# intel/hdk

Measured on AMD Instinct MI355X. Metric: rows/sec, 1B-row int64 GROUP BY SUM, higher is better.
Workload: dtype int64; 1 GPU; C2: SELECT key, SUM(val) GROUP BY key; int64, 64 uniform keys; rows=1000000000, rows_per_gpu=1000000000, fragments=32, fragments_per_gpu=32, fragment_rows=32000000, layout=perfect hash, keyless, 64 entries, parallelism=fragment f -> GPU f mod 1; one GPU

## Files before the change

### hdk_amd/_lib.py

```python
import ctypes as C
import os
import subprocess

from . import _abi as A

_HERE = os.path.dirname(os.path.abspath(__file__))
LIB_PATH = os.environ.get("HDK_HIP_LIB") or os.path.join(_HERE, "libhdk_hip.so")
CSRC = os.path.join(_HERE, "csrc")


class HdkHipError(RuntimeError):
    def __init__(self, code, msg):
        super().__init__(f"hdk_hip status {code}: {msg}")
        self.code = code


def build(force=False):
    if force:
        subprocess.check_call(["make", "-C", CSRC, "clean"])
    subprocess.check_call(["make", "-C", CSRC, "-j4"])
    return LIB_PATH


_lib = None
# ... 116 lines not shown
                          f"{LIB_PATH} is missing: run `python -c 'import __graft_entry__ as g; g.build()'` "
                          "(make -C hdk_amd/csrc).  There is no CPU fallback.")
    _share_hip_runtime_with_torch()
    L = C.CDLL(LIB_PATH)
    for name, (res, args) in {**SIGNATURES, **EXTRA_SIGNATURES}.items():
        f = getattr(L, name)
        f.restype = res
        f.argtypes = args
    _lib = L
    return L


_switch_env = None


def sync_switches():
    global _switch_env
    now = tuple(sorted((k, v) for k, v in os.environ.items() if k.startswith("HDK_HIP_")))
    if now != _switch_env:
        lib().hdk_hip_reload_switches()
        _switch_env = now


def check(status: int):
    if status != A.OK:
        msg = lib().hdk_hip_last_error()
        raise HdkHipError(status, msg.decode() if msg else "")
    return status
```

### hdk_amd/csrc/host_common.h

```cpp
#pragma once
#include <hip/hip_runtime.h>
#include <stdarg.h>
#include <stdint.h>
#include <stdio.h>

#include "../../include/hdk_hip.h"

namespace hdk {

void set_error(const char* fmt, ...);
void clear_error();
int32_t device_enter(int32_t device_id, void* stream, hipStream_t* out);
const hdk_hip_device_properties* device_props(int32_t device_id);
const int32_t* device_interrupt_word(int32_t device_id);
enum ScanPer { SCAN_PER_4 = 4, SCAN_PER_16 = 16 };
void launch_counts_scan(uint32_t* counts, uint32_t n, ScanPer per, uint64_t* total_out, hipStream_t s);
int32_t launch_init_row_wise_indirect(int64_t* const* groupby_buf, const int64_t* init_vals, uint32_t entry_count,
                                      uint32_t key_count, uint32_t key_width, uint32_t row_size_quad, int keyless,
                                      const hdk_hip_device_properties* props, hipStream_t s);
inline int32_t init_row_wise_output(const hdk_hip_plan* plan, int64_t* const* groupby_buf, const int64_t* init_vals,
                                    const hdk_hip_device_properties* props, hipStream_t s) {
  const uint32_t key_count = plan->keyless ? 0u : static_cast<uint32_t>(plan->key_count);
  return launch_init_row_wise_indirect(groupby_buf, init_vals, plan->entry_count, key_count, static_cast<uint32_t>(plan->key_width),
                                       plan->row_size_quad, plan->keyless, props, s);
}

#define HDK_HIP_CHECK(expr)                                                                  \
  do {                                                                                       \
    hipError_t e_ = (expr);                                                                  \
    if (e_ != hipSuccess) {                                                                  \
      hdk::set_error("%s failed: %s (%s:%d)", #expr, hipGetErrorString(e_), __FILE__, __LINE__); \
      return e_ == hipErrorOutOfMemory ? HDK_HIP_ERR_OUT_OF_GPU_MEM : HDK_HIP_ERR_RUNTIME;   \
    }                                                                                        \
  } while (0)

#define HDK_REQUIRE(cond, ...)          \
  do {                                  \
// ... 51 lines not shown
```

### hdk_amd/csrc/reduce.hip

```cpp
#include <mutex>
#include <string.h>

#include "baseline_table.h"
#include "device_common.h"
#include "group_buffer.h"
#include "host_common.h"

namespace hdk {

constexpr int kPlanCacheSlots = 16;
struct PlanCacheEntry {
  hdk_hip_plan host;
  hdk_hip_plan* dev = nullptr;
  bool used = false;
};
struct PlanCache {
  std::mutex mu;
  PlanCacheEntry e[kPlanCacheSlots];
  int next = 0;
};
static PlanCache g_plan_cache[16];

static int32_t cached_device_plan(const hdk_hip_plan* plan, int32_t device_id, const hdk_hip_plan** out) {
  PlanCache& c = g_plan_cache[device_id & 15];
  std::lock_guard<std::mutex> lk(c.mu);
  for (int i = 0; i < kPlanCacheSlots; ++i) {
    if (c.e[i].used && memcmp(&c.e[i].host, plan, sizeof(hdk_hip_plan)) == 0) {
      *out = c.e[i].dev;
      return HDK_HIP_OK;
    }
  }
  PlanCacheEntry& e = c.e[c.next];
  c.next = (c.next + 1) % kPlanCacheSlots;
  if (!e.dev) {
    HDK_HIP_CHECK(hipMalloc(reinterpret_cast<void**>(&e.dev), sizeof(hdk_hip_plan)));
  }
  e.used = false;
  HDK_HIP_CHECK(hipDeviceSynchronize());
  HDK_HIP_CHECK(hipMemcpy(e.dev, plan, sizeof(hdk_hip_plan), hipMemcpyHostToDevice));
  memcpy(&e.host, plan, sizeof(hdk_hip_plan));
  e.used = true;
  *out = e.dev;
  return HDK_HIP_OK;
}

constexpr int kRedBlock = 256;
HDK_DEV bool reduce_single_value(const hdk_hip_target& tg, int8_t* this1, const int8_t* that1, int64_t init_val) {
  if (tg.slot_width == 4) {
    const int32_t l = *reinterpret_cast<const int32_t*>(this1), r = *reinterpret_cast<const int32_t*>(that1);
    if (r == static_cast<int32_t>(init_val)) return false;
    if (l == static_cast<int32_t>(init_val)) {
      *reinterpret_cast<int32_t*>(this1) = r;
      return false;
    }
    return l != r;
  }
  const int64_t l = *reinterpret_cast<const int64_t*>(this1), r = *reinterpret_cast<const int64_t*>(that1);
  if (r == init_val) return false;
  if (l == init_val) {
    *reinterpret_cast<int64_t*>(this1) = r;
    return false;
  }
  return l != r;
}

HDK_DEV void reduce_slot(const hdk_hip_target& tg, int8_t* this1, int8_t* this2, const int8_t* that1,
                         const int8_t* that2, int64_t init_val) {
// ... 356 lines not shown
    nslots += p->targets[t].agg == HDK_AGG_AVG ? 2 : 1;
  }
  size_t off = p->keyless ? 0 : static_cast<size_t>(p->key_count) * ((static_cast<size_t>(entry_count) * 8 + 7) & ~size_t(7));
  int s = 0;
  for (int t = 0; t < p->num_targets && s < nslots; ++t) {
    off = (off + 7) & ~size_t(7);
    off += static_cast<size_t>(entry_count) * p->targets[t].slot_width;
    ++s;
    if (p->targets[t].agg == HDK_AGG_AVG) {
      off = (off + 7) & ~size_t(7);
      off += static_cast<size_t>(entry_count) * p->targets[t].slot2_width;
      ++s;
    }
  }
  return ((off + 7) & ~size_t(7)) / 8;
}

template <int MODE>
static int32_t run_partition(const hdk_hip_plan* plan, const int64_t* buf, uint32_t entry_count, const int64_t* init_vals,
                             int32_t num_owners, uint32_t* counts_out, const OwnerSegs& segs, int32_t device_id,
                             hipStream_t s) {
  SlotInit init;
  fill_slot_init(plan, init_vals, &init);
  AsyncScratch mem(s);
  constexpr size_t kPlanBytes = align256(sizeof(hdk_hip_plan));
  HDK_HIP_CHECK(hipMallocAsync(&mem.p, kPlanBytes + kMaxOwners * sizeof(uint32_t), s));
  int8_t* scratch = static_cast<int8_t*>(mem.p);
  hdk_hip_plan* d_plan = reinterpret_cast<hdk_hip_plan*>(scratch);
  uint32_t* cursors = reinterpret_cast<uint32_t*>(scratch + kPlanBytes);
  HDK_HIP_CHECK(hipMemcpyAsync(d_plan, plan, sizeof(hdk_hip_plan), hipMemcpyHostToDevice, s));
  HDK_HIP_CHECK(hipMemsetAsync(cursors, 0, kMaxOwners * sizeof(uint32_t), s));
  const hdk_hip_device_properties* props = device_props(device_id);
  unsigned blocks = persistent_grid(props, (static_cast<size_t>(entry_count) + kRedBlock * kPartT - 1) / (kRedBlock * kPartT));
  if (blocks == 0) blocks = 1;
  const bool k32 = !plan->output_columnar && plan->key_width == 4;
  if (k32) {
    hipLaunchKernelGGL((k_partition_baseline<int32_t, MODE>), dim3(blocks), dim3(kRedBlock), 0, s,
                       d_plan, buf, entry_count, static_cast<uint32_t>(num_owners), init, cursors, segs);
  } else {
    hipLaunchKernelGGL((k_partition_baseline<int64_t, MODE>), dim3(blocks), dim3(kRedBlock), 0, s,
                       d_plan, buf, entry_count, static_cast<uint32_t>(num_owners), init, cursors, segs);
  }
  HDK_HIP_CHECK(hipGetLastError());
  if (counts_out) {
    HDK_HIP_CHECK(hipMemcpyAsync(counts_out, cursors, num_owners * sizeof(uint32_t), hipMemcpyDeviceToHost, s));
    HDK_HIP_CHECK(hipStreamSynchronize(s));
  }
  return HDK_HIP_OK;
}

int32_t validate_plan_layout(const hdk_hip_plan* p);

}
// ... 118 lines not shown
```

### hdk_amd/csrc/runtime.hip

```cpp
#include <algorithm>
#include <mutex>
#include <stdlib.h>
#include <string.h>

#include "host_common.h"
#include "switches.h"

namespace hdk {
namespace {
constexpr int kSwitchLen = 64;
const char* const kSwitchNames[SW_COUNT] = {
#define HDK_SW_NAME(name) "HDK_HIP_" #name,
    HDK_SWITCH_LIST(HDK_SW_NAME)
#undef HDK_SW_NAME
};
struct SwitchTable {
  bool set[SW_COUNT];
  char val[SW_COUNT][kSwitchLen];
};
SwitchTable g_switches;
std::once_flag g_switches_once;
void read_switches() {
  for (int i = 0; i < SW_COUNT; ++i) {
    const char* e = getenv(kSwitchNames[i]);
// ... 93 lines not shown
  std::call_once(g_dev[d].once, init_device, d);
  if (g_dev[d].status != HDK_HIP_OK) {
    set_error("failed to initialise device %d", d);
  }
  return g_dev[d].status;
}

int32_t device_enter(int32_t device_id, void* stream, hipStream_t* out) {
  const int32_t st = ensure_device(device_id);
  if (st != HDK_HIP_OK) {
    return st;
  }
  HDK_HIP_CHECK(hipSetDevice(device_id));
  *out = stream ? static_cast<hipStream_t>(stream) : g_dev[device_id].stream;
  return HDK_HIP_OK;
}

const hdk_hip_device_properties* device_props(int32_t device_id) {
  return ensure_device(device_id) == HDK_HIP_OK ? &g_dev[device_id].props : nullptr;
}

const int32_t* device_interrupt_word(int32_t device_id) {
  return ensure_device(device_id) == HDK_HIP_OK ? g_dev[device_id].interrupt_word : nullptr;
}

}

using namespace hdk;

extern "C" int32_t hdk_hip_set_interrupt(int32_t device_id, int32_t value) {
  hipStream_t main_stream;
  const int32_t st = device_enter(device_id, nullptr, &main_stream);
  if (st) return st;
  DeviceState& d = g_dev[device_id];
  std::lock_guard<std::mutex> lk(d.interrupt_mu);
  HDK_HIP_CHECK(hipMemcpyAsync(d.interrupt_word, &value, sizeof(int32_t), hipMemcpyHostToDevice, d.interrupt_stream));
  HDK_HIP_CHECK(hipStreamSynchronize(d.interrupt_stream));
  return HDK_HIP_OK;
}

extern "C" {

const char* hdk_hip_last_error(void) { return tl_error; }
int32_t hdk_hip_version(void) { return 1004; }

int32_t hdk_hip_mgr_get_device_count(int32_t* count) {
// ... 289 lines not shown
```

### hdk_amd/csrc/scan_agg.hip

```cpp
#include "agg_common.h"
#include "watch.h"

namespace hdk {

constexpr int kBlock = 256;

HDK_DEV void lds_add_u64(int64_t* p, int64_t v) {
  atomicAdd(reinterpret_cast<unsigned long long*>(p), static_cast<unsigned long long>(v));
}
HDK_DEV void lds_add_f64(int64_t* p, double v) {
  atomicAdd(reinterpret_cast<double*>(p), v);
}
HDK_DEV void lds_min_i64(int64_t* p, int64_t v) { atomicMin(reinterpret_cast<long long*>(p), static_cast<long long>(v)); }
HDK_DEV void lds_max_i64(int64_t* p, int64_t v) { atomicMax(reinterpret_cast<long long*>(p), static_cast<long long>(v)); }
HDK_DEV void lds_min_f64(int64_t* p, double v) {
  unsigned long long* a = reinterpret_cast<unsigned long long*>(p);
  unsigned long long old = *a;
  while (v < bits_to_double(static_cast<int64_t>(old))) {
    const unsigned long long assumed = old;
    old = atomicCAS(a, assumed, static_cast<unsigned long long>(double_to_bits(v)));
    if (old == assumed) {
      break;
    }
  }
// ... 116 lines not shown
    int64_t acc = lds[i * rep];
    for (uint32_t r = 1; r < rep; ++r) {
      acc = word_combine(op, acc, lds[i * rep + r]);
    }
    if (wl.is_nword[i % wpe]) {
      const uint32_t w0 = (i / wpe) * wpe;
      int64_t rows = 0;
      for (uint32_t r = 0; r < rep; ++r) {
        rows += lds[w0 * rep + r];
      }
      acc = rows - acc;
    }
    slab[i] = acc;
  }
}

struct FinalizeArgs {
  const hdk_hip_plan* plan;
  const int64_t* slabs;
  int64_t** groupby_buf;
  uint32_t num_slabs;
  uint32_t entry_count;
  const uint32_t* skip_if;
};

HDK_DEV int64_t shfl_down_i64(int64_t v, int delta) {
  int lo = static_cast<int>(v & 0xffffffff);
  int hi = static_cast<int>(v >> 32);
  lo = __shfl_down(lo, delta, kWave);
  hi = __shfl_down(hi, delta, kWave);
  return (static_cast<int64_t>(hi) << 32) | static_cast<uint32_t>(lo);
}

HDK_DEV void apply_count(int8_t* slot, int width, int64_t cnt) {
  if (width == 4) {
    *reinterpret_cast<int32_t*>(slot) =
        static_cast<int32_t>(static_cast<uint32_t>(*reinterpret_cast<int32_t*>(slot)) + static_cast<uint32_t>(cnt));
  } else {
    *reinterpret_cast<int64_t*>(slot) =
        static_cast<int64_t>(static_cast<uint64_t>(*reinterpret_cast<int64_t*>(slot)) + static_cast<uint64_t>(cnt));
  }
}

HDK_DEV void apply_value(const hdk_hip_target& tg, int8_t* slot, int64_t partial, int64_t nn, int64_t rowcount) {
  const bool skip = tg.skip_null;
  if ((skip && nn == 0) || rowcount == 0) {
// ... 48 lines not shown
  }
  if (tg.arg_is_fp) {
    const double o = bits_to_double(old);
    const double v = bits_to_double(partial);
    double r;
    if (agg == HDK_AGG_MIN) {
      r = (v < o) ? v : o;
    } else if (agg == HDK_AGG_MAX) {
      r = (o < v) ? v : o;
    } else {
      r = o + v;
    }
    *s = double_to_bits(r);
  } else if (agg == HDK_AGG_MIN) {
    *s = old < partial ? old : partial;
  } else if (agg == HDK_AGG_MAX) {
    *s = old > partial ? old : partial;
  } else {
    *s = static_cast<int64_t>(static_cast<uint64_t>(old) + static_cast<uint64_t>(partial));
  }
}

HDK_DEV void finalize_apply(const hdk_hip_plan* __restrict__ p, const WordLayout& wl, const FinalizeArgs& a, uint32_t entry,
                            const int64_t* words, int ws) {
  const int64_t rowcount = words[0];
  if (rowcount == 0) {
    return;
  }
  int64_t* buf = a.groupby_buf[0];
  const bool grouped = p->query_kind != HDK_Q_NON_GROUPED;
  const bool columnar = p->output_columnar;
  const int nk = p->key_count;
  int64_t keys[HDK_HIP_MAX_KEYS];
  if (grouped) {
    uint64_t rem = entry;
#pragma unroll
    for (int k = 0; k < HDK_HIP_MAX_KEYS; ++k) {
      if (k < nk) {
        uint64_t comp = rem;
        if (nk > 1) {
          comp = rem % static_cast<uint64_t>(p->key_card[k]);
          rem /= static_cast<uint64_t>(p->key_card[k]);
        }
        const int64_t bucket = p->key_bucket[k] ? p->key_bucket[k] : 1;
        keys[k] = p->key_min[k] + static_cast<int64_t>(comp) * bucket;
      }
    }
    if (!p->keyless) {
      if (columnar) {
        if (buf[entry] == HDK_EMPTY_KEY_64) {
#pragma unroll
          for (int k = 0; k < HDK_HIP_MAX_KEYS; ++k) {
            if (k < nk) {
              buf[static_cast<size_t>(k) * a.entry_count + entry] = keys[k];
            }
          }
        }
      } else {
        int64_t* row = buf + static_cast<size_t>(entry) * p->row_size_quad;
        if (row[0] == HDK_EMPTY_KEY_64) {
#pragma unroll
          for (int k = 0; k < HDK_HIP_MAX_KEYS; ++k) {
            if (k < nk) {
              row[k] = keys[k];
            }
          }
        }
      }
    }
  }
  const int nt = p->num_targets;
  int slot_idx = 0;
  for (int t = 0; t < nt; ++t) {
    const hdk_hip_target& tg = p->targets[t];
    int8_t* s1;
    int8_t* s2 = nullptr;
    if (!grouped) {
      s1 = reinterpret_cast<int8_t*>(a.groupby_buf[slot_idx]);
      if (tg.agg == HDK_AGG_AVG) {
        s2 = reinterpret_cast<int8_t*>(a.groupby_buf[slot_idx + 1]);
      }
    } else if (columnar) {
      s1 = reinterpret_cast<int8_t*>(buf) + columnar_slot_off(p, a.entry_count, slot_idx) +
           static_cast<size_t>(entry) * tg.slot_width;
      if (tg.agg == HDK_AGG_AVG) {
        s2 = reinterpret_cast<int8_t*>(buf) + columnar_slot_off(p, a.entry_count, slot_idx + 1) +
             static_cast<size_t>(entry) * tg.slot2_width;
      }
    } else {
      int8_t* row = reinterpret_cast<int8_t*>(buf + static_cast<size_t>(entry) * p->row_size_quad);
      s1 = row + tg.slot_off;
      s2 = row + tg.slot2_off;
    }
    const int vw = wl.vword[t];
    const int nw = wl.nword[t];
    const int64_t nn = nw >= 0 ? words[nw * ws] : rowcount;
    switch (tg.agg) {
      case HDK_AGG_COUNT:
        apply_count(s1, tg.slot_width, nn);
        break;
      case HDK_AGG_ID: {
        int64_t kv = keys[0];
#pragma unroll
        for (int k = 1; k < HDK_HIP_MAX_KEYS; ++k) {
          if (k == tg.key_idx) {
            kv = keys[k];
          }
        }
        const int ki = tg.key_idx;
        if (p->key_has_nulls[ki] && kv == p->key_null_translated[ki]) {
          kv = p->keys[ki].null_val;
        }
        if (tg.slot_width == 4) {
          *reinterpret_cast<int32_t*>(s1) = static_cast<int32_t>(kv);
        } else {
          *reinterpret_cast<int64_t*>(s1) = kv;
        }
        break;
      }
      case HDK_AGG_AVG:
        apply_count(s2, tg.slot2_width, nn);
        apply_value(tg, s1, words[vw * ws], nn, rowcount);
        break;
      default:
        apply_value(tg, s1, words[vw * ws], nn, rowcount);
        break;
    }
    slot_idx += tg.agg == HDK_AGG_AVG ? 2 : 1;
  }
}


extern "C" __global__ __launch_bounds__(kBlock) void hdk_finalize(FinalizeArgs a) {
  __shared__ WordLayout wl;
  __shared__ int64_t s_words[kBlock / kWave][kMaxWordsPerEntry];
  const hdk_hip_plan* __restrict__ p = a.plan;
  if (a.skip_if && *a.skip_if) {
    return;
  }
  if (threadIdx.x == 0) {
    make_word_layout(p, &wl);
  }
  __syncthreads();
  const int lane = threadIdx.x & (kWave - 1);
  const uint32_t entry = blockIdx.x * (kBlock / kWave) + (threadIdx.x / kWave);
  if (entry >= a.entry_count) {
    return;
  }
  const int wpe = wl.wpe;
  const size_t ew = static_cast<size_t>(a.entry_count) * wpe;
  int64_t* words = s_words[threadIdx.x / kWave];
  for (int w = 0; w < wpe; ++w) {
    const int32_t op = wl.wop[w];
    int64_t acc = word_identity(op);
    for (uint32_t b = lane; b < a.num_slabs; b += kWave) {
      acc = word_combine(op, acc, a.slabs[b * ew + static_cast<size_t>(entry) * wpe + w]);
    }
    for (int d = kWave / 2; d > 0; d >>= 1) {
      acc = word_combine(op, acc, shfl_down_i64(acc, d));
    }
    if (lane == 0) {
      words[w] = acc;
    }
  }
  if (lane != 0) {
    return;
  }
  finalize_apply(p, wl, a, entry, words, 1);
}

constexpr int kFinalizeFlatBlock = 256;
extern "C" __global__ __launch_bounds__(kFinalizeFlatBlock) void hdk_finalize_flat(FinalizeArgs a) {
  __shared__ WordLayout wl;
  __shared__ int64_t s_words[kMaxWordsPerEntry][kFinalizeFlatBlock];
  const hdk_hip_plan* __restrict__ p = a.plan;
  if (a.skip_if && *a.skip_if) {
    return;
  }
  if (threadIdx.x == 0) {
    make_word_layout(p, &wl);
  }
  __syncthreads();
  const uint32_t entry = blockIdx.x * kFinalizeFlatBlock + threadIdx.x;
  if (entry >= a.entry_count) {
    return;
  }
  const int wpe = wl.wpe;
  const size_t ew = static_cast<size_t>(a.entry_count) * wpe;
  for (int w = 0; w < wpe; ++w) {
    const int32_t op = wl.wop[w];
    int64_t acc = word_identity(op);
    for (uint32_t b = 0; b < a.num_slabs; ++b) {
      acc = word_combine(op, acc, a.slabs[b * ew + static_cast<size_t>(entry) * wpe + w]);
    }
    s_words[w][threadIdx.x] = acc;
  }
  finalize_apply(p, wl, a, entry, &s_words[0][threadIdx.x], kFinalizeFlatBlock);
}

}

#include <mutex>
#include <utility>
#include <vector>

#include <stddef.h>
#include <string.h>

#include "host_match.h"
#include "scan_bh_host.h"
#include "scan_bhm_host.h"
#include "scan_agg_fast.h"
#include "scan_agg_cols.h"
#include "scan_agg_vec.h"
#include "scan_agg_keys.h"
#include "scan_cluster.h"
// ... 229 lines not shown
static uint32_t keys_lds_bytes(const KeysArgs& ka, const LaunchShape& shape) {
  return ka.nvals ? shape.lds_bytes : shape.lds_bytes / 2;
}
static const void* keys_kernel(const KeysArgs& ka, uint32_t block = kKeysBlock) {
  int wmax = 1;
  for (int k = 0; k < ka.nkeys; ++k) wmax = ka.key[k].width > wmax ? ka.key[k].width : wmax;
  for (int v = 0; v < ka.nvals; ++v) wmax = ka.val[v].width > wmax ? ka.val[v].width : wmax;
  if (ka.nvals && block == kKeysWideBlock) {
    return wmax == 8 ? reinterpret_cast<const void*>(hdk_scan_agg_keys<true, 2, kKeysWideBlock>)
                     : reinterpret_cast<const void*>(hdk_scan_agg_keys<true, 4, kKeysWideBlock>);
  }
  if (ka.nvals) {
    return wmax == 8 ? reinterpret_cast<const void*>(hdk_scan_agg_keys<true, 2>)
                     : reinterpret_cast<const void*>(hdk_scan_agg_keys<true, 4>);
  }
  return wmax == 8 ? reinterpret_cast<const void*>(hdk_scan_agg_keys<false, 2>)
                   : reinterpret_cast<const void*>(hdk_scan_agg_keys<false, 4>);
}


__global__ void k_arm_watch(LaunchWatch* w, uint32_t flags, uint32_t watchdog_ms) {
  w->flags = flags;
  w->deadline = __builtin_amdgcn_s_memrealtime() + static_cast<uint64_t>(watchdog_ms) * 100000ull;
}

static LaunchShape base_shape(const hdk_hip_plan* p, const hdk_hip_kernel_options* ko, const hdk_hip_device_properties* props) {
  LaunchShape s;
  WordLayout wl;
  make_word_layout(p, &wl);
  s.wpe = wl.wpe;
  s.entry_count = p->query_kind == HDK_Q_NON_GROUPED ? 1u : p->entry_count;
  s.grid = (ko && ko->grid_dim_x) ? ko->grid_dim_x : static_cast<uint32_t>(props->grid_size);
  s.block = kBlock;
  bool force_global = ko && (ko->flags & HDK_HIP_LAUNCH_FORCE_GLOBAL_ATOMICS);
  for (int t = 0; t < p->num_targets; ++t) {
    force_global = force_global || p->targets[t].agg == HDK_AGG_SINGLE_VALUE;
  }
  const uint64_t words = static_cast<uint64_t>(s.entry_count) * s.wpe;
  if (p->query_kind == HDK_Q_PROJECTION) {
    s.strategy = STRAT_PROJECT;
    s.rep = 1;
    s.lds_bytes = 0;
    s.slab_words = 0;
  } else if (p->query_kind != HDK_Q_BASELINE_HASH && words <= kLdsMaxTableWords && !force_global) {
    s.strategy = STRAT_LDS;
    uint32_t rep = 32;
// ... 1368 lines not shown
    if (kk.xf != KXF_NONE && kk.col_nullable) {
      bool null_is_fast;
      if (kk.xf == KXF_YEAR) {
        null_is_fast = static_cast<uint64_t>(kk.col_null) <= static_cast<uint64_t>(UINT32_MAX - 2208988800u);
      } else {
        const uint64_t half = static_cast<uint64_t>(kk.param >> 1);
        const int64_t tmp = static_cast<int64_t>(kk.col_null >= 0 ? static_cast<uint64_t>(kk.col_null) + half
                                                                  : static_cast<uint64_t>(kk.col_null) - half);
        const int32_t t32 = static_cast<int32_t>(tmp);
        null_is_fast = t32 == tmp && t32 != INT32_MIN;
      }
      if (null_is_fast) return false;
    }
    if (shape.entry_count >= kKeysPoison) return false;
  }
  return true;
}

int32_t launch_head(const hdk_hip_plan* plan, int8_t* const params[HDK_KP_COUNT], const hdk_hip_kernel_options* ko,
                    int32_t device_id, void* workspace, hipStream_t s, hdk_hip_plan** d_plan_out, KernParams* kp_out) {
  hdk_hip_plan* d_plan = static_cast<hdk_hip_plan*>(workspace);
  *d_plan_out = d_plan;
  LaunchWatch* d_watch = reinterpret_cast<LaunchWatch*>(static_cast<int8_t*>(workspace) + kWatchOffset);
  const bool plan_resident = ko && (ko->flags & HDK_HIP_LAUNCH_PLAN_RESIDENT);
  if (!plan_resident) {
    struct alignas(16) Head {
      int8_t bytes[kWatchOffset + sizeof(LaunchWatch)];
    } head;
    static_assert(sizeof(LaunchWatch) == 16, "LaunchWatch is 16 bytes");
    memcpy(head.bytes, plan, sizeof(hdk_hip_plan));
    memset(head.bytes + sizeof(hdk_hip_plan), 0, sizeof(head.bytes) - sizeof(hdk_hip_plan));
    HDK_HIP_CHECK(hipMemcpyAsync(d_plan, head.bytes, sizeof(head.bytes), hipMemcpyHostToDevice, s));
  }
  {
    const uint32_t wf = ((ko && (ko->flags & HDK_HIP_LAUNCH_CHECK_INTERRUPT)) ? 1u : 0u) | ((ko && ko->watchdog_ms) ? 2u : 0u);
    if (wf || plan_resident) {
      hipLaunchKernelGGL(k_arm_watch, dim3(1), dim3(1), 0, s, d_watch, wf, ko ? ko->watchdog_ms : 0u);
      HDK_HIP_CHECK(hipGetLastError());
    }
  }

  KernParams& kp = *kp_out;
  kp.col_buffers = reinterpret_cast<const int8_t* const* const*>(params[HDK_KP_COL_BUFFERS]);
  kp.num_fragments = reinterpret_cast<const uint64_t*>(params[HDK_KP_NUM_FRAGMENTS]);
  kp.literals = params[HDK_KP_LITERALS];
  kp.num_rows = reinterpret_cast<const int64_t*>(params[HDK_KP_NUM_ROWS]);
  kp.frag_row_offsets = reinterpret_cast<const uint64_t*>(params[HDK_KP_FRAG_ROW_OFFSETS]);
  kp.max_matched = reinterpret_cast<const int32_t*>(params[HDK_KP_MAX_MATCHED]);
  kp.total_matched = reinterpret_cast<int32_t*>(params[HDK_KP_TOTAL_MATCHED]);
  kp.init_agg_vals = reinterpret_cast<const int64_t*>(params[HDK_KP_INIT_AGG_VALS]);
  kp.groupby_buf = reinterpret_cast<int64_t**>(params[HDK_KP_GROUPBY_BUF]);
  kp.error_code = reinterpret_cast<int32_t*>(params[HDK_KP_ERROR_CODE]);
  kp.num_tables = reinterpret_cast<const uint32_t*>(params[HDK_KP_NUM_TABLES]);
  kp.join_hash_tables = reinterpret_cast<const int64_t*>(params[HDK_KP_JOIN_HASH_TABLES]);
  kp.watch = d_watch;
  kp.interrupt = device_interrupt_word(device_id);

  return HDK_HIP_OK;
}

}

extern "C" int32_t hdk_hip_validate_plan(const hdk_hip_plan* plan, int32_t layout_only) {
// ... 71 lines not shown
  ca.num_fragments = reinterpret_cast<uint64_t*>(q);
  ca.kp = *kp;
  const size_t lds = static_cast<size_t>(kClusterTile) * ca.ncols * 8 + kClusterTile + 16;
  unsigned grid = resident_grid(reinterpret_cast<const void*>(hdk_cluster_by_key), kClusterBlock, lds, props);
  hipLaunchKernelGGL(hdk_cluster_by_key, dim3(grid), dim3(kClusterBlock), lds, s, ca);
  hipLaunchKernelGGL(hdk_cluster_params, dim3(8), dim3(256), 0, s, ca);
  HDK_HIP_CHECK(hipGetLastError());
  kp->col_buffers = reinterpret_cast<const int8_t* const* const*>(ca.frag_ptrs);
  kp->num_fragments = ca.num_fragments;
  kp->num_rows = ca.num_rows;
  kp->frag_row_offsets = ca.frag_offs;
  return HDK_HIP_OK;
}

int32_t hdk::launch_finalize_slabs(const hdk_hip_plan* d_plan, const int64_t* slabs, int64_t** groupby_buf, uint32_t num_slabs,
                                   uint32_t entry_count, const uint32_t* skip_if, hipStream_t s) {
  FinalizeArgs fa;
  fa.plan = d_plan;
  fa.slabs = slabs;
  fa.groupby_buf = groupby_buf;
  fa.num_slabs = num_slabs;
  fa.entry_count = entry_count;
  fa.skip_if = skip_if;
  if (num_slabs <= 16 && entry_count >= 2048) {
    hipLaunchKernelGGL(hdk_finalize_flat, dim3((entry_count + kFinalizeFlatBlock - 1) / kFinalizeFlatBlock), dim3(kFinalizeFlatBlock), 0, s, fa);
    HDK_HIP_CHECK(hipGetLastError());
    return HDK_HIP_OK;
  }
  const unsigned fblocks = (entry_count + (kBlock / kWave) - 1) / (kBlock / kWave);
  hipLaunchKernelGGL(hdk_finalize, dim3(fblocks), dim3(kBlock), 0, s, fa);
  HDK_HIP_CHECK(hipGetLastError());
  return HDK_HIP_OK;
}

static void route_launch(const hdk_hip_plan* p, const hdk_hip_kernel_options* ko, const hdk_hip_device_properties* props, RouteSet refused,
                         LaunchRoute* r) {
  r->pre = PRE_NONE;
  r->shape = base_shape(p, ko, props);
  if (r->shape.strategy == STRAT_PROJECT) {
    route_project(p, ko, props, r);
  } else if (r->shape.strategy == STRAT_GLOBAL) {
    route_baseline(p, ko, props, refused, r);
  } else {
    route_scan_lds(p, ko, props, refused, r);
    const void* const k = r->as<const void*>();
    if (r->kind == ROUTE_VEC && p->query_kind == HDK_Q_PERFECT_HASH && !route_bh_packed(p, ko, refused, r)) {
      r->kind = ROUTE_VEC;
      r->as<const void*>() = k;
    }
  }
  if (!route_clusters_its_own_input(r->kind) && match_cluster_join(p, ko, &r->pre_as<ClusterArgs>())) r->pre = PRE_CLUSTER_BY_KEY;
}

static int32_t launch_route(LaunchRoute& r, const hdk_hip_plan* plan, const hdk_hip_plan* d_plan, const KernParams& kp, int64_t* slabs,
                            const hdk_hip_kernel_options* ko, bool* init_output, const hdk_hip_device_properties* props, hipStream_t s,
                            bool* launched) {
  if (r.shape.strategy == STRAT_PROJECT) {
    *launched = true;
    return launch_project(r, plan, d_plan, kp, ko, props, s);
  }
  if (r.shape.strategy == STRAT_GLOBAL) return launch_baseline(r, plan, d_plan, kp, ko, init_output, props, s, launched);
  if (*init_output) {
    const int32_t st = init_row_wise_output(plan, kp.groupby_buf, kp.init_agg_vals, props, s);
    if (st) return st;
    *init_output = false;
  }
  if (!route_fills_slabs(r.kind)) return launch_bh_packed(r, plan, d_plan, kp, ko, props, s, launched);
  return launch_scan_lds(r, plan, d_plan, kp, slabs, ko, props, s, launched);
}

extern "C" int32_t hdk_hip_workspace_size(const hdk_hip_plan* plan, const hdk_hip_kernel_options* ko,
                                          int32_t device_id, size_t* bytes) {
  HDK_REQUIRE(bytes, "bytes is NULL");
  const int32_t st = validate_plan(plan);
  if (st) return st;
  const hdk_hip_device_properties* props = device_props(device_id);
  if (!props) return HDK_HIP_ERR_RUNTIME;
  LaunchRoute r;
  route_launch(plan, ko, props, 0, &r);
  *bytes = workspace_bytes_for(r.shape);
  return HDK_HIP_OK;
}

extern "C" int32_t hdk_hip_describe_launch(const hdk_hip_plan* plan, const hdk_hip_kernel_options* ko,
                                           int32_t device_id, char* out, size_t out_len) {
  HDK_REQUIRE(out && out_len, "out is NULL");
  const int32_t st = validate_plan(plan);
  if (st) return st;
  static const hdk_hip_device_properties assumed = [] {
    hdk_hip_device_properties p;
    memset(&p, 0, sizeof(p));
    p.global_mem = 288ull << 30;
    p.num_cu = 256;
    p.max_threads_per_block = 1024;
    p.wavefront_size = 64;
    p.grid_size = 4 * 256;
    p.shared_mem_per_block = 160 << 10;
    p.has_shared_memory_atomics = p.can_load_async = p.has_fp64 = 1;
    strncpy(p.arch_name, "gfx950 (assumed)", sizeof(p.arch_name) - 1);
    return p;
  }();
  const hdk_hip_device_properties* props = device_id == HDK_HIP_DEVICE_ASSUMED_MI355X ? &assumed : device_props(device_id);
  if (!props) return HDK_HIP_ERR_RUNTIME;
  LaunchRoute r;
  route_launch(plan, ko, props, 0, &r);
  snprintf(out, out_len, "%s%s", r.pre == PRE_CLUSTER_BY_KEY ? "hdk_cluster_by_key,hdk_cluster_params," : "", route_info(r.kind).kernels);
  return HDK_HIP_OK;
}

extern "C" int32_t hdk_hip_launch(const hdk_hip_plan* plan, int8_t* const params[HDK_KP_COUNT],
                                  const hdk_hip_kernel_options* ko, int32_t device_id, void* stream,
                                  void* workspace, size_t workspace_bytes) {
  int32_t st = validate_plan(plan);
  if (st) return st;
  HDK_REQUIRE(params, "params is NULL");
  HDK_REQUIRE(params[HDK_KP_NUM_FRAGMENTS] && params[HDK_KP_NUM_ROWS] && params[HDK_KP_NUM_TABLES] &&
                  params[HDK_KP_GROUPBY_BUF] && params[HDK_KP_ERROR_CODE],
              "a required kernel parameter is NULL");
  HDK_REQUIRE(plan->num_joins == 0 || params[HDK_KP_JOIN_HASH_TABLES], "JOIN_HASH_TABLES is NULL");
  HDK_REQUIRE(plan->query_kind == HDK_Q_PROJECTION || params[HDK_KP_INIT_AGG_VALS], "INIT_AGG_VALS is NULL");
  HDK_REQUIRE(plan->query_kind != HDK_Q_PROJECTION || (params[HDK_KP_MAX_MATCHED] && params[HDK_KP_TOTAL_MATCHED]),
              "MAX_MATCHED / TOTAL_MATCHED is NULL");
  hipStream_t s;
  st = device_enter(device_id, stream, &s);
  if (st) return st;
  const hdk_hip_device_properties* props = device_props(device_id);
  LaunchRoute r;
  route_launch(plan, ko, props, 0, &r);
  const LaunchShape& shape = r.shape;
// ... 40 lines not shown
    st = launch_cluster_join(r.pre_as<ClusterArgs>(), &kp, props, s, &cluster_scratch.p);
    if (st) return st;
  }
  int64_t* slabs = reinterpret_cast<int64_t*>(static_cast<int8_t*>(workspace) + kPlanRegionBytes);
  for (RouteSet refused = 0;;) {
    bool launched = false;
    st = launch_route(r, plan, d_plan, kp, slabs, ko, &init_output, props, s, &launched);
    if (st) return st;
    if (launched) break;
    refused |= RouteSet(1) << r.kind;
    route_launch(plan, ko, props, refused, &r);
  }
  if (timed) {
    HDK_HIP_CHECK(hipEventRecord(e1, s));
  }
  if (route_fills_slabs(r.kind)) {
    FinalizeArgs fa;
    fa.skip_if = nullptr;
    fa.plan = d_plan;
    fa.slabs = slabs;
    fa.groupby_buf = kp.groupby_buf;
    fa.num_slabs = shape.grid;
    fa.entry_count = shape.entry_count;
    const unsigned fblocks = (shape.entry_count + (kBlock / kWave) - 1) / (kBlock / kWave);
    hipLaunchKernelGGL(hdk_finalize, dim3(fblocks), dim3(kBlock), 0, s, fa);
    HDK_HIP_CHECK(hipGetLastError());
  }
  return HDK_HIP_OK;
}

extern "C" int32_t hdk_hip_collect_scan_times(int32_t device_id, float* ms_out, int32_t capacity, int32_t* count) {
  HDK_REQUIRE(count, "count is NULL");
  HDK_REQUIRE(device_id >= 0 && device_id < 16, "bad device");
  std::lock_guard<std::mutex> lk(g_scan_events[device_id].mu);
  auto& v = g_scan_events[device_id].pending;
  int32_t n = 0;
  for (auto& pr : v) {
    HDK_HIP_CHECK(hipEventSynchronize(pr.second));
    float ms = 0.f;
    HDK_HIP_CHECK(hipEventElapsedTime(&ms, pr.first, pr.second));
    if (ms_out && n < capacity) {
      ms_out[n] = ms;
    }
    ++n;
    (void)hipEventDestroy(pr.first);
    (void)hipEventDestroy(pr.second);
// ... 6 lines not shown
```

### hdk_amd/executor.py

```python
import ctypes as C
import dataclasses
from typing import Dict, List, Optional

import numpy as np

from . import _abi as A
from . import result_set
from ._lib import HdkHipError, check, lib, sync_switches
from .hip_mgr import DeviceBuffer, HipMgr
from .ir import QueryMustRunOnCpu, QueryUnit
from .plan import (DEFAULT_MAX_GROUPS_BUFFER_ENTRY_GUESS, GROUP_KINDS, ColumnDesc, CompiledPlan, Having, columnar_init_vals,
                   compact_init_vals, compile_query, describe_columns, eff_key_count, has_count_distinct, regroup_columns,
                   resolve_having, resolve_having_columns, resolve_order_by, split_count_distinct)
from .storage import ArrowStorage


class BufferCache:

    def __init__(self, mgr: HipMgr, device_id: int):
        self.mgr, self.device_id = mgr, device_id
        self._chunks: Dict[tuple, DeviceBuffer] = {}

    def chunk(self, table, col_name, frag_idx) -> DeviceBuffer:
        key = (table.name, col_name, frag_idx)
        b = self._chunks.get(key)
        if b is None:
            b = self.mgr.to_device(table.columns[col_name].fragments[frag_idx], self.device_id)
            self._chunks[key] = b
        return b

    def linearized(self, table, col_name) -> DeviceBuffer:
# ... 234 lines not shown
            out.block, out.capacity, out.num_rows = sized_columns(self.mgr, self.device_id, len(spec), n, call,
                                                                  self.GROUP_ONE_CALL_BYTES, drop_empty=True)
        finally:
            if src is not self:
                src.free()
        return out

    def free(self):
        if self.block is not None:
            self.block.free()
            self.block = None


class PreparedStep:

    def __init__(self, ex: "Executor", cp: CompiledPlan, frag_ids: List[int], grid=0, flags=0,
                 out_ptr: Optional[int] = None, watchdog_ms: int = 0):
        self.ex, self.cp, self.frag_ids = ex, cp, list(frag_ids)
        self.mgr, self.dev = ex.mgr, ex.device_id
        self.L = lib()
        sync_switches()
        self.keep: List[DeviceBuffer] = []
        self._graph = None
        p = cp.plan
        storage = ex.storage
        outer = storage.get(cp.query.table)
        nfrag = len(self.frag_ids)
        self.rows_in_step = int(sum(outer.frag_rows[f] for f in self.frag_ids))
        self.ko = A.KernelOptions(grid, 0, 0, flags, self.rows_in_step, int(watchdog_ms), 0)
        ntab = 1 + len(cp.inner_tables)

        self.plan = A.Plan.from_buffer_copy(cp.plan)
        fuse = bool(cp.inner_tables) and ex.fuse_join_tables and \
            not (flags & (A.LAUNCH_FORCE_SCALAR | A.LAUNCH_FORCE_GLOBAL_ATOMICS)) and \
            bool({"hdk_scan_agg_vec_join", "hdk_scan_project_join", "hdk_scan_agg_vec_keyed", "hdk_scan_project_keyed",
                  "hdk_scan_agg_bh_vec_join"} &
                 set(self.kernel_names().split(",")))
        self.join_tables = []
        for ji in range(len(cp.inner_tables)):
            spec = self._fuse_spec(ji) if fuse else None
            self.join_tables.append(ex._build_join_table(cp, ji, ((spec[0], self), spec[1], spec[2]) if spec else None))
        if fuse:
            self._fuse_join_tables()
        p = self.plan

        ncols = len(cp.input_cols)
# ... 149 lines not shown
                self.out_ptr, self.d_init_raw.ptr, p.entry_count, eff_key_count(p), len(self.cp.slot_widths),
                self.d_col_sizes.ptr, 1, p.keyless, 8, props.max_threads_per_block, props.grid_size,
                self.dev, stream))
        else:
            check(self.L.hdk_hip_init_group_by_buffer(
                self.out_ptr, self.d_init.ptr, p.entry_count, eff_key_count(p), p.key_width, p.row_size_quad,
                p.keyless, 1, props.max_threads_per_block, props.grid_size, self.dev, stream))
        if p.query_kind == A.Q_PROJECTION:
            check(self.L.hdk_hip_init_group_by_buffer(
                self.d_total_matched.ptr, self.d_zero.ptr, 1, 0, 8, 1, 1, 1,
                props.max_threads_per_block, props.grid_size, self.dev, stream))

    def launch(self, stream=None, init_output=False):
        ko = self.ko
        if init_output:
            ko = A.KernelOptions.from_buffer_copy(self.ko)
            ko.flags |= A.LAUNCH_INIT_OUTPUT
        check(self.L.hdk_hip_launch(C.byref(self.plan), self._params, C.byref(ko), self.dev, stream,
                                    self.workspace.ptr, self.workspace.nbytes))

    @property
    def launch_initialises(self) -> bool:
        p = self.cp.plan
        return p.query_kind == A.Q_BASELINE_HASH and not p.output_columnar

    def enqueue(self, stream=None):
        if self.launch_initialises:
            self.launch(stream, init_output=True)
        else:
            self.init_output(stream)
            self.launch(stream)

    def fetch(self, stream_synced=False) -> ExecutionResult:
        if not stream_synced:
            self.mgr.synchronizeStream(self.dev)
        err = int(self.mgr.to_host(self.d_err.ptr, 4, self.dev, np.int32)[0])
        if err > 0:
            raise HdkHipError(err, f"device error code {err} (QE/Execute.h:1019-1031)")
        buf = self.mgr.to_host(self.out_ptr, max(self.buffer_bytes, 8), self.dev, np.int64)
        total = None
        if self.cp.plan.query_kind == A.Q_PROJECTION:
            total = int(self.mgr.to_host(self.d_total_matched.ptr, 4, self.dev, np.int32)[0])
        return ExecutionResult(self.cp, buf[:self.buffer_bytes // 8], self.cp.entry_count, err, total)

    COLUMNS_ONE_CALL_BYTES = ONE_CALL_BYTES

    def fetch_columns(self, stream_synced=False) -> DeviceColumns:
        if not stream_synced:
            self.mgr.synchronizeStream(self.dev)
        err = int(self.mgr.to_host(self.d_err.ptr, 4, self.dev, np.int32)[0])
        if err > 0:
            raise HdkHipError(err, f"device error code {err} (QE/Execute.h:1019-1031)")
        p = self.cp.plan
        n, nt = int(self.cp.entry_count), int(p.num_targets)
        iv = np.ascontiguousarray(self.cp.init_vals, dtype=np.int64)

        def call(out_ptr, capacity, row_count_ptr):
            check(self.L.hdk_hip_columnarize_result(C.byref(p), self.out_ptr, n, iv.ctypes.data, out_ptr, capacity,
                                                    row_count_ptr, None, 0, self.dev, None))

        block, capacity, rows = sized_columns(self.mgr, self.dev, nt, n, call, self.COLUMNS_ONE_CALL_BYTES)
        return DeviceColumns(self.cp, self.mgr, self.dev, block, capacity, rows, err)

    def run(self, stream=None) -> ExecutionResult:
        self.enqueue(stream)
        return self.fetch()

    def capture_graph(self, stream=None):
        if self._graph or not self.kernel_names().endswith("hdk_finalize"):
            return self
        self.init_output(stream)
        self.launch(stream)
        self.mgr.synchronizeStream(self.dev) if stream is None else None
        saved = self.ko.flags
        self.ko.flags = (saved | A.LAUNCH_PLAN_RESIDENT) & ~A.LAUNCH_RECORD_EVENTS
        try:
            check(self.L.hdk_hip_graph_begin_capture(self.dev, stream))
            self.init_output(stream)
            self.launch(stream)
            g = C.c_void_p()
            check(self.L.hdk_hip_graph_end_capture(self.dev, stream, C.byref(g)))
            self._graph = g
        finally:
            self.ko.flags = saved
        return self

    def replay(self, stream=None):
        if self._graph:
            check(self.L.hdk_hip_graph_launch(self._graph, self.dev, stream))
        else:
            self.enqueue(stream)

    def free(self):
        if self._graph:
            self.L.hdk_hip_graph_destroy(self._graph)
            self._graph = None
        for b in self.keep:
            b.free()
        self.keep.clear()


class Executor:
# ... 185 lines not shown
```

Baseline: 432.5 billion rows/s.

## Fuse output init into finalize and cache device plans across launches

Moves the device plan cache into the runtime and shares it across launches. The launch head now copies the cached device plan with a small kernel instead of doing a host-to-device memcpy on every launch. For perfect-hash slab routes, output initialisation is folded into hdk_finalize: rows are built in shared memory and written once, so the separate init kernel is no longer needed. The finalize slab loops are also unrolled over several slabs and words to keep more loads in flight. The cost is extra complexity, a possible hipDeviceSynchronize when the cache evicts an entry, and reliance on describe_launch to decide whether init is fused.

```diff
diff --git a/hdk_amd/_lib.py b/hdk_amd/_lib.py
--- a/hdk_amd/_lib.py
+++ b/hdk_amd/_lib.py
@@ -162,6 +162,10 @@
         _switch_env = now
 
 
+def switch_state():
+    return _switch_env
+
+
 def check(status: int):
     if status != A.OK:
         msg = lib().hdk_hip_last_error()
diff --git a/hdk_amd/csrc/host_common.h b/hdk_amd/csrc/host_common.h
--- a/hdk_amd/csrc/host_common.h
+++ b/hdk_amd/csrc/host_common.h
@@ -13,6 +13,7 @@
 int32_t device_enter(int32_t device_id, void* stream, hipStream_t* out);
 const hdk_hip_device_properties* device_props(int32_t device_id);
 const int32_t* device_interrupt_word(int32_t device_id);
+int32_t cached_device_plan(const hdk_hip_plan* plan, int32_t device_id, const hdk_hip_plan** out);
 enum ScanPer { SCAN_PER_4 = 4, SCAN_PER_16 = 16 };
 void launch_counts_scan(uint32_t* counts, uint32_t n, ScanPer per, uint64_t* total_out, hipStream_t s);
 int32_t launch_init_row_wise_indirect(int64_t* const* groupby_buf, const int64_t* init_vals, uint32_t entry_count,
diff --git a/hdk_amd/csrc/reduce.hip b/hdk_amd/csrc/reduce.hip
--- a/hdk_amd/csrc/reduce.hip
+++ b/hdk_amd/csrc/reduce.hip
@@ -7,42 +7,6 @@
 #include "host_common.h"
 
 namespace hdk {
-
-constexpr int kPlanCacheSlots = 16;
-struct PlanCacheEntry {
-  hdk_hip_plan host;
-  hdk_hip_plan* dev = nullptr;
-  bool used = false;
-};
-struct PlanCache {
-  std::mutex mu;
-  PlanCacheEntry e[kPlanCacheSlots];
-  int next = 0;
-};
-static PlanCache g_plan_cache[16];
-
-static int32_t cached_device_plan(const hdk_hip_plan* plan, int32_t device_id, const hdk_hip_plan** out) {
-  PlanCache& c = g_plan_cache[device_id & 15];
-  std::lock_guard<std::mutex> lk(c.mu);
-  for (int i = 0; i < kPlanCacheSlots; ++i) {
-    if (c.e[i].used && memcmp(&c.e[i].host, plan, sizeof(hdk_hip_plan)) == 0) {
-      *out = c.e[i].dev;
-      return HDK_HIP_OK;
-    }
-  }
-  PlanCacheEntry& e = c.e[c.next];
-  c.next = (c.next + 1) % kPlanCacheSlots;
-  if (!e.dev) {
-    HDK_HIP_CHECK(hipMalloc(reinterpret_cast<void**>(&e.dev), sizeof(hdk_hip_plan)));
-  }
-  e.used = false;
-  HDK_HIP_CHECK(hipDeviceSynchronize());
-  HDK_HIP_CHECK(hipMemcpy(e.dev, plan, sizeof(hdk_hip_plan), hipMemcpyHostToDevice));
-  memcpy(&e.host, plan, sizeof(hdk_hip_plan));
-  e.used = true;
-  *out = e.dev;
-  return HDK_HIP_OK;
-}
 
 constexpr int kRedBlock = 256;
 HDK_DEV bool reduce_single_value(const hdk_hip_target& tg, int8_t* this1, const int8_t* that1, int64_t init_val) {
@@ -445,13 +409,12 @@
                              hipStream_t s) {
   SlotInit init;
   fill_slot_init(plan, init_vals, &init);
+  const hdk_hip_plan* d_plan = nullptr;
+  const int32_t st = cached_device_plan(plan, device_id, &d_plan);
+  if (st) return st;
   AsyncScratch mem(s);
-  constexpr size_t kPlanBytes = align256(sizeof(hdk_hip_plan));
-  HDK_HIP_CHECK(hipMallocAsync(&mem.p, kPlanBytes + kMaxOwners * sizeof(uint32_t), s));
-  int8_t* scratch = static_cast<int8_t*>(mem.p);
-  hdk_hip_plan* d_plan = reinterpret_cast<hdk_hip_plan*>(scratch);
-  uint32_t* cursors = reinterpret_cast<uint32_t*>(scratch + kPlanBytes);
-  HDK_HIP_CHECK(hipMemcpyAsync(d_plan, plan, sizeof(hdk_hip_plan), hipMemcpyHostToDevice, s));
+  HDK_HIP_CHECK(hipMallocAsync(&mem.p, kMaxOwners * sizeof(uint32_t), s));
+  uint32_t* cursors = static_cast<uint32_t*>(mem.p);
   HDK_HIP_CHECK(hipMemsetAsync(cursors, 0, kMaxOwners * sizeof(uint32_t), s));
   const hdk_hip_device_properties* props = device_props(device_id);
   unsigned blocks = persistent_grid(props, (static_cast<size_t>(entry_count) + kRedBlock * kPartT - 1) / (kRedBlock * kPartT));
diff --git a/hdk_amd/csrc/runtime.hip b/hdk_amd/csrc/runtime.hip
--- a/hdk_amd/csrc/runtime.hip
+++ b/hdk_amd/csrc/runtime.hip
@@ -139,6 +139,54 @@
 
 const int32_t* device_interrupt_word(int32_t device_id) {
   return ensure_device(device_id) == HDK_HIP_OK ? g_dev[device_id].interrupt_word : nullptr;
+}
+
+constexpr int kPlanCacheSlots = 64;
+struct PlanCache {
+  std::mutex mu;
+  hdk_hip_plan* host = nullptr;
+  hdk_hip_plan* dev = nullptr;
+  bool used[kPlanCacheSlots] = {};
+  int next = 0;
+  int last = 0;
+};
+static PlanCache g_plan_cache[kMaxDevices];
+
+int32_t cached_device_plan(const hdk_hip_plan* plan, int32_t device_id, const hdk_hip_plan** out) {
+  if (device_id < 0 || device_id >= kMaxDevices) {
+    set_error("device %d out of range", device_id);
+    return HDK_HIP_ERR_INVALID_ARG;
+  }
+  PlanCache& c = g_plan_cache[device_id];
+  std::lock_guard<std::mutex> lk(c.mu);
+  if (!c.dev) {
+    c.host = static_cast<hdk_hip_plan*>(malloc(sizeof(hdk_hip_plan) * kPlanCacheSlots));
+    if (!c.host) {
+      set_error("out of host memory for the plan cache");
+      return HDK_HIP_ERR_RUNTIME;
+    }
+    HDK_HIP_CHECK(hipMalloc(reinterpret_cast<void**>(&c.dev), sizeof(hdk_hip_plan) * kPlanCacheSlots));
+  }
+  for (int k = 0; k < kPlanCacheSlots; ++k) {
+    const int i = (c.last + k) % kPlanCacheSlots;
+    if (c.used[i] && memcmp(&c.host[i], plan, sizeof(hdk_hip_plan)) == 0) {
+      c.last = i;
+      *out = c.dev + i;
+      return HDK_HIP_OK;
+    }
+  }
+  const int i = c.next;
+  if (c.used[i]) {
+    c.used[i] = false;
+    HDK_HIP_CHECK(hipDeviceSynchronize());
+  }
+  HDK_HIP_CHECK(hipMemcpy(c.dev + i, plan, sizeof(hdk_hip_plan), hipMemcpyHostToDevice));
+  memcpy(&c.host[i], plan, sizeof(hdk_hip_plan));
+  c.used[i] = true;
+  c.next = (i + 1) % kPlanCacheSlots;
+  c.last = i;
+  *out = c.dev + i;
+  return HDK_HIP_OK;
 }
 
 }
diff --git a/hdk_amd/csrc/scan_agg.hip b/hdk_amd/csrc/scan_agg.hip
--- a/hdk_amd/csrc/scan_agg.hip
+++ b/hdk_amd/csrc/scan_agg.hip
@@ -162,6 +162,8 @@
   uint32_t num_slabs;
   uint32_t entry_count;
   const uint32_t* skip_if;
+  const int64_t* init_vals;
+  uint32_t fresh;
 };
 
 HDK_DEV int64_t shfl_down_i64(int64_t v, int delta) {
@@ -256,12 +258,21 @@
 }
 
 HDK_DEV void finalize_apply(const hdk_hip_plan* __restrict__ p, const WordLayout& wl, const FinalizeArgs& a, uint32_t entry,
-                            const int64_t* words, int ws) {
+                            const int64_t* words, int ws, int64_t* staged = nullptr) {
   const int64_t rowcount = words[0];
+  int64_t* buf = a.groupby_buf[0];
+  if (a.fresh && !staged) {
+    const uint32_t rq = p->row_size_quad;
+    const uint32_t key_count = p->keyless ? 0u : static_cast<uint32_t>(p->key_count);
+    const uint32_t keys_quads = p->keyless ? 0u : (key_count * static_cast<uint32_t>(p->key_width) + 7) / 8;
+    int64_t* row = buf + static_cast<size_t>(entry) * rq;
+    for (uint32_t q = 0; q < rq; ++q) {
+      row[q] = init_row_quad(q, keys_quads, key_count, static_cast<uint32_t>(p->key_width), a.init_vals);
+    }
+  }
   if (rowcount == 0) {
     return;
   }
-  int64_t* buf = a.groupby_buf[0];
   const bool grouped = p->query_kind != HDK_Q_NON_GROUPED;
   const bool columnar = p->output_columnar;
   const int nk = p->key_count;
@@ -291,8 +302,8 @@
           }
         }
       } else {
-        int64_t* row = buf + static_cast<size_t>(entry) * p->row_size_quad;
-        if (row[0] == HDK_EMPTY_KEY_64) {
+        int64_t* row = staged ? staged : buf + static_cast<size_t>(entry) * p->row_size_quad;
+        if (a.fresh || row[0] == HDK_EMPTY_KEY_64) {
 #pragma unroll
           for (int k = 0; k < HDK_HIP_MAX_KEYS; ++k) {
             if (k < nk) {
@@ -322,7 +333,7 @@
              static_cast<size_t>(entry) * tg.slot2_width;
       }
     } else {
-      int8_t* row = reinterpret_cast<int8_t*>(buf + static_cast<size_t>(entry) * p->row_size_quad);
+      int8_t* row = reinterpret_cast<int8_t*>(staged ? staged : buf + static_cast<size_t>(entry) * p->row_size_quad);
       s1 = row + tg.slot_off;
       s2 = row + tg.slot2_off;
     }
@@ -365,15 +376,28 @@
 }
 
 
+constexpr int kFinWords = 4;
+constexpr int kFinSlabs = 8;
+static_assert(kBlock >= 2 * kWave, "hdk_finalize: the second wave builds the init image");
+constexpr uint32_t kFreshRowQuads = 32;
 extern "C" __global__ __launch_bounds__(kBlock) void hdk_finalize(FinalizeArgs a) {
   __shared__ WordLayout wl;
   __shared__ int64_t s_words[kBlock / kWave][kMaxWordsPerEntry];
+  __shared__ int64_t s_row[kBlock / kWave + 1][kFreshRowQuads];
   const hdk_hip_plan* __restrict__ p = a.plan;
   if (a.skip_if && *a.skip_if) {
     return;
   }
+  const uint32_t rq = p->row_size_quad;
+  const bool stage = a.fresh && rq <= kFreshRowQuads;
   if (threadIdx.x == 0) {
     make_word_layout(p, &wl);
+  }
+  if (stage && threadIdx.x >= kWave && threadIdx.x - kWave < rq) {
+    const uint32_t key_count = p->keyless ? 0u : static_cast<uint32_t>(p->key_count);
+    const uint32_t keys_quads = p->keyless ? 0u : (key_count * static_cast<uint32_t>(p->key_width) + 7) / 8;
+    s_row[kBlock / kWave][threadIdx.x - kWave] =
+        init_row_quad(threadIdx.x - kWave, keys_quads, key_count, static_cast<uint32_t>(p->key_width), a.init_vals);
   }
   __syncthreads();
   const int lane = threadIdx.x & (kWave - 1);
@@ -384,26 +408,68 @@
   const int wpe = wl.wpe;
   const size_t ew = static_cast<size_t>(a.entry_count) * wpe;
   int64_t* words = s_words[threadIdx.x / kWave];
-  for (int w = 0; w < wpe; ++w) {
-    const int32_t op = wl.wop[w];
-    int64_t acc = word_identity(op);
-    for (uint32_t b = lane; b < a.num_slabs; b += kWave) {
-      acc = word_combine(op, acc, a.slabs[b * ew + static_cast<size_t>(entry) * wpe + w]);
-    }
-    for (int d = kWave / 2; d > 0; d >>= 1) {
-      acc = word_combine(op, acc, shfl_down_i64(acc, d));
-    }
-    if (lane == 0) {
-      words[w] = acc;
+  const int64_t* const src = a.slabs + static_cast<size_t>(entry) * wpe;
+  for (int w0 = 0; w0 < wpe; w0 += kFinWords) {
+    int32_t op[kFinWords];
+    int64_t acc[kFinWords];
+#pragma unroll
+    for (int j = 0; j < kFinWords; ++j) {
+      op[j] = wl.wop[w0 + j < wpe ? w0 + j : wpe - 1];
+      acc[j] = word_identity(op[j]);
+    }
+    for (uint32_t b0 = lane; b0 < a.num_slabs; b0 += kWave * kFinSlabs) {
+      int64_t v[kFinSlabs][kFinWords];
+#pragma unroll
+      for (int u = 0; u < kFinSlabs; ++u) {
+        const uint32_t b = b0 + u * kWave;
+#pragma unroll
+        for (int j = 0; j < kFinWords; ++j) {
+          v[u][j] = (b < a.num_slabs && w0 + j < wpe) ? src[b * ew + w0 + j] : 0;
+        }
+      }
+#pragma unroll
+      for (int u = 0; u < kFinSlabs; ++u) {
+        const uint32_t b = b0 + u * kWave;
+#pragma unroll
+        for (int j = 0; j < kFinWords; ++j) {
+          if (b < a.num_slabs && w0 + j < wpe) {
+            acc[j] = word_combine(op[j], acc[j], v[u][j]);
+          }
+        }
+      }
+    }
+#pragma unroll
+    for (int j = 0; j < kFinWords; ++j) {
+      if (w0 + j < wpe) {
+        for (int d = kWave / 2; d > 0; d >>= 1) {
+          acc[j] = word_combine(op[j], acc[j], shfl_down_i64(acc[j], d));
+        }
+        if (lane == 0) {
+          words[w0 + j] = acc[j];
+        }
+      }
     }
   }
   if (lane != 0) {
     return;
   }
-  finalize_apply(p, wl, a, entry, words, 1);
+  if (!stage) {
+    finalize_apply(p, wl, a, entry, words, 1);
+    return;
+  }
+  int64_t* staged = s_row[threadIdx.x / kWave];
+  for (uint32_t q = 0; q < rq; ++q) {
+    staged[q] = s_row[kBlock / kWave][q];
+  }
+  finalize_apply(p, wl, a, entry, words, 1, staged);
+  int64_t* row = a.groupby_buf[0] + static_cast<size_t>(entry) * rq;
+  for (uint32_t q = 0; q < rq; ++q) {
+    row[q] = staged[q];
+  }
 }
 
 constexpr int kFinalizeFlatBlock = 256;
+constexpr int kFinFlatSlabs = 16;
 extern "C" __global__ __launch_bounds__(kFinalizeFlatBlock) void hdk_finalize_flat(FinalizeArgs a) {
   __shared__ WordLayout wl;
   __shared__ int64_t s_words[kMaxWordsPerEntry][kFinalizeFlatBlock];
@@ -424,8 +490,19 @@
   for (int w = 0; w < wpe; ++w) {
     const int32_t op = wl.wop[w];
     int64_t acc = word_identity(op);
-    for (uint32_t b = 0; b < a.num_slabs; ++b) {
-      acc = word_combine(op, acc, a.slabs[b * ew + static_cast<size_t>(entry) * wpe + w]);
+    const int64_t* const src = a.slabs + static_cast<size_t>(entry) * wpe + w;
+    for (uint32_t b0 = 0; b0 < a.num_slabs; b0 += kFinFlatSlabs) {
+      int64_t v[kFinFlatSlabs];
+#pragma unroll
+      for (int u = 0; u < kFinFlatSlabs; ++u) {
+        v[u] = b0 + u < a.num_slabs ? src[(b0 + u) * ew] : 0;
+      }
+#pragma unroll
+      for (int u = 0; u < kFinFlatSlabs; ++u) {
+        if (b0 + u < a.num_slabs) {
+          acc = word_combine(op, acc, v[u]);
+        }
+      }
     }
     s_words[w][threadIdx.x] = acc;
   }
@@ -701,6 +778,22 @@
 __global__ void k_arm_watch(LaunchWatch* w, uint32_t flags, uint32_t watchdog_ms) {
   w->flags = flags;
   w->deadline = __builtin_amdgcn_s_memrealtime() + static_cast<uint64_t>(watchdog_ms) * 100000ull;
+}
+
+constexpr int kHeadBlock = 256;
+static_assert(sizeof(hdk_hip_plan) % 8 == 0 && alignof(hdk_hip_plan) >= 8, "the plan is copied in 8-byte words");
+__global__ __launch_bounds__(kHeadBlock) void k_launch_head(const hdk_hip_plan* __restrict__ src, hdk_hip_plan* __restrict__ dst,
+                                                            LaunchWatch* w, uint32_t flags, uint32_t watchdog_ms) {
+  const uint64_t* __restrict__ s8 = reinterpret_cast<const uint64_t*>(src);
+  uint64_t* __restrict__ d8 = reinterpret_cast<uint64_t*>(dst);
+  for (uint32_t i = threadIdx.x; i < sizeof(hdk_hip_plan) / 8; i += kHeadBlock) {
+    d8[i] = s8[i];
+  }
+  if (threadIdx.x == 0) {
+    w->flags = flags;
+    w->pad_ = 0;
+    w->deadline = __builtin_amdgcn_s_memrealtime() + static_cast<uint64_t>(watchdog_ms) * 100000ull;
+  }
 }
 
 static LaunchShape base_shape(const hdk_hip_plan* p, const hdk_hip_kernel_options* ko, const hdk_hip_device_properties* props) {
@@ -2115,23 +2208,18 @@
   hdk_hip_plan* d_plan = static_cast<hdk_hip_plan*>(workspace);
   *d_plan_out = d_plan;
   LaunchWatch* d_watch = reinterpret_cast<LaunchWatch*>(static_cast<int8_t*>(workspace) + kWatchOffset);
+  static_assert(sizeof(LaunchWatch) == 16, "LaunchWatch is 16 bytes");
   const bool plan_resident = ko && (ko->flags & HDK_HIP_LAUNCH_PLAN_RESIDENT);
-  if (!plan_resident) {
-    struct alignas(16) Head {
-      int8_t bytes[kWatchOffset + sizeof(LaunchWatch)];
-    } head;
-    static_assert(sizeof(LaunchWatch) == 16, "LaunchWatch is 16 bytes");
-    memcpy(head.bytes, plan, sizeof(hdk_hip_plan));
-    memset(head.bytes + sizeof(hdk_hip_plan), 0, sizeof(head.bytes) - sizeof(hdk_hip_plan));
-    HDK_HIP_CHECK(hipMemcpyAsync(d_plan, head.bytes, sizeof(head.bytes), hipMemcpyHostToDevice, s));
-  }
-  {
-    const uint32_t wf = ((ko && (ko->flags & HDK_HIP_LAUNCH_CHECK_INTERRUPT)) ? 1u : 0u) | ((ko && ko->watchdog_ms) ? 2u : 0u);
-    if (wf || plan_resident) {
-      hipLaunchKernelGGL(k_arm_watch, dim3(1), dim3(1), 0, s, d_watch, wf, ko ? ko->watchdog_ms : 0u);
-      HDK_HIP_CHECK(hipGetLastError());
-    }
-  }
+  const uint32_t wf = ((ko && (ko->flags & HDK_HIP_LAUNCH_CHECK_INTERRUPT)) ? 1u : 0u) | ((ko && ko->watchdog_ms) ? 2u : 0u);
+  if (plan_resident) {
+    hipLaunchKernelGGL(k_arm_watch, dim3(1), dim3(1), 0, s, d_watch, wf, ko ? ko->watchdog_ms : 0u);
+  } else {
+    const hdk_hip_plan* c_plan = nullptr;
+    const int32_t st = cached_device_plan(plan, device_id, &c_plan);
+    if (st) return st;
+    hipLaunchKernelGGL(k_launch_head, dim3(1), dim3(kHeadBlock), 0, s, c_plan, d_plan, d_watch, wf, ko ? ko->watchdog_ms : 0u);
+  }
+  HDK_HIP_CHECK(hipGetLastError());
 
   KernParams& kp = *kp_out;
   kp.col_buffers = reinterpret_cast<const int8_t* const* const*>(params[HDK_KP_COL_BUFFERS]);
@@ -2249,6 +2337,8 @@
   fa.num_slabs = num_slabs;
   fa.entry_count = entry_count;
   fa.skip_if = skip_if;
+  fa.init_vals = nullptr;
+  fa.fresh = 0;
   if (num_slabs <= 16 && entry_count >= 2048) {
     hipLaunchKernelGGL(hdk_finalize_flat, dim3((entry_count + kFinalizeFlatBlock - 1) / kFinalizeFlatBlock), dim3(kFinalizeFlatBlock), 0, s, fa);
     HDK_HIP_CHECK(hipGetLastError());
@@ -2287,7 +2377,7 @@
     return launch_project(r, plan, d_plan, kp, ko, props, s);
   }
   if (r.shape.strategy == STRAT_GLOBAL) return launch_baseline(r, plan, d_plan, kp, ko, init_output, props, s, launched);
-  if (*init_output) {
+  if (*init_output && !route_fills_slabs(r.kind)) {
     const int32_t st = init_row_wise_output(plan, kp.groupby_buf, kp.init_agg_vals, props, s);
     if (st) return st;
     *init_output = false;
@@ -2331,7 +2421,10 @@
   if (!props) return HDK_HIP_ERR_RUNTIME;
   LaunchRoute r;
   route_launch(plan, ko, props, 0, &r);
-  snprintf(out, out_len, "%s%s", r.pre == PRE_CLUSTER_BY_KEY ? "hdk_cluster_by_key,hdk_cluster_params," : "", route_info(r.kind).kernels);
+  const bool init_kernel = ko && (ko->flags & HDK_HIP_LAUNCH_INIT_OUTPUT) && r.shape.strategy != STRAT_PROJECT &&
+                           !route_fills_slabs(r.kind) && r.kind != ROUTE_RADIX_PARTITIONED;
+  snprintf(out, out_len, "%s%s%s", init_kernel ? "k_init_row_wise_indirect," : "",
+           r.pre == PRE_CLUSTER_BY_KEY ? "hdk_cluster_by_key,hdk_cluster_params," : "", route_info(r.kind).kernels);
   return HDK_HIP_OK;
 }
 
@@ -2418,6 +2511,8 @@
     fa.groupby_buf = kp.groupby_buf;
     fa.num_slabs = shape.grid;
     fa.entry_count = shape.entry_count;
+    fa.init_vals = kp.init_agg_vals;
+    fa.fresh = init_output ? 1u : 0u;
     const unsigned fblocks = (shape.entry_count + (kBlock / kWave) - 1) / (kBlock / kWave);
     hipLaunchKernelGGL(hdk_finalize, dim3(fblocks), dim3(kBlock), 0, s, fa);
     HDK_HIP_CHECK(hipGetLastError());
diff --git a/hdk_amd/executor.py b/hdk_amd/executor.py
--- a/hdk_amd/executor.py
+++ b/hdk_amd/executor.py
@@ -6,7 +6,7 @@
 
 from . import _abi as A
 from . import result_set
-from ._lib import HdkHipError, check, lib, sync_switches
+from ._lib import HdkHipError, check, lib, switch_state, sync_switches
 from .hip_mgr import DeviceBuffer, HipMgr
 from .ir import QueryMustRunOnCpu, QueryUnit
 from .plan import (DEFAULT_MAX_GROUPS_BUFFER_ENTRY_GUESS, GROUP_KINDS, ColumnDesc, CompiledPlan, Having, columnar_init_vals,
@@ -287,6 +287,7 @@
         sync_switches()
         self.keep: List[DeviceBuffer] = []
         self._graph = None
+        self._fused_init = None
         p = cp.plan
         storage = ex.storage
         outer = storage.get(cp.query.table)
@@ -482,7 +483,18 @@
     @property
     def launch_initialises(self) -> bool:
         p = self.cp.plan
-        return p.query_kind == A.Q_BASELINE_HASH and not p.output_columnar
+        if p.output_columnar or p.query_kind not in (A.Q_PERFECT_HASH, A.Q_BASELINE_HASH):
+            return False
+        if p.query_kind == A.Q_BASELINE_HASH:
+            return True
+        key = (int(self.ko.flags), int(self.ko.grid_dim_x), switch_state())
+        if self._fused_init is None or self._fused_init[0] != key:
+            ko = A.KernelOptions.from_buffer_copy(self.ko)
+            ko.flags |= A.LAUNCH_INIT_OUTPUT
+            out = C.create_string_buffer(256)
+            check(self.L.hdk_hip_describe_launch(C.byref(self.plan), C.byref(ko), self.dev, out, 256))
+            self._fused_init = (key, not out.value.decode().startswith("k_init_row_wise"))
+        return self._fused_init[1]
 
     def enqueue(self, stream=None):
         if self.launch_initialises:
@@ -529,15 +541,13 @@
     def capture_graph(self, stream=None):
         if self._graph or not self.kernel_names().endswith("hdk_finalize"):
             return self
-        self.init_output(stream)
-        self.launch(stream)
+        self.enqueue(stream)
         self.mgr.synchronizeStream(self.dev) if stream is None else None
         saved = self.ko.flags
         self.ko.flags = (saved | A.LAUNCH_PLAN_RESIDENT) & ~A.LAUNCH_RECORD_EVENTS
         try:
             check(self.L.hdk_hip_graph_begin_capture(self.dev, stream))
-            self.init_output(stream)
-            self.launch(stream)
+            self.enqueue(stream)
             g = C.c_void_p()
             check(self.L.hdk_hip_graph_end_capture(self.dev, stream, C.byref(g)))
             self._graph = g
```

New measurement: 432.2 billion rows/s. Within noise of the previous version (-0.1%).
